# fema-ffrd/gpras

Hardware: AMD Instinct MI355X
Metric: gp_fits_per_sec (higher is better)
Workload: dtype f64; 1 GPU; BASELINE configs[1] as the many-independent-cells workload: exact GP N=4096 d=8 RBF, fit F1 = kernel build + blocked fp64-MFMA Cholesky + alpha + LML, per cell; cells = y columns of one training set with per-cell hyperparameters (the reference's per-mode models); n_train=4096, d=8, kernel=RBF, collective=none (one process), launcher=single process

## Files before the change

### gpras_amd/_lib.py

```python

from __future__ import annotations

import ctypes as C
from pathlib import Path

import numpy as np

import os

LIB_PATH = Path(os.environ["GPRX_LIBRARY"]) if os.environ.get("GPRX_LIBRARY") else Path(__file__).resolve().parent / "libgprx.so"

GPRX_OK, GPRX_EINVAL, GPRX_ENOTPD, GPRX_EHIP, GPRX_ENOMEM, GPRX_ESTATE, GPRX_ERCCL, GPRX_ENOCONV = range(8)
UNIQUE_ID_BYTES = 128
TRAIN_VARIANCE, TRAIN_LENGTHSCALE, TRAIN_NOISE, TRAIN_Z = 1, 2, 4, 8
GEMM_C_LOWER, GEMM_A_LOWER, GEMM_A_UPPER, GEMM_B_LOWER, GEMM_B_UPPER = 1, 2, 4, 8, 16
REDUCE_LOGDET_QUAD, REDUCE_COL, REDUCE_ROWSQ_FINAL, REDUCE_ROW = range(4)

DISTANCE_FORMS = {"difference": 0, "expanded": 1}
KERNEL_IDS = {"RBF": 0, "Matern12": 1, "Matern32": 2, "Matern52": 3, "Exponential": 4}


class GprxLibraryError(RuntimeError):
    """libgprx.so is missing or unusable."""

# ... 96 lines not shown
    "gprx_api": (C.c_int, [C.c_int, _vp, _i64, _vp, _i64, _i64, _vp]),
    "gprx_spline_eval": (C.c_int, [C.c_int, _vp, C.c_int, _vp, _vp, _i64, _vp]),
    "gprx_ps_create": (C.c_int, [C.c_int, _i64, _vp, _vp, _i64, _vp, _vp, C.c_int, _vp, _vp, C.c_int, _vp, C.POINTER(_vp)]),
    "gprx_ps_destroy": (C.c_int, [_vp]),
    "gprx_ps_last_error": (C.c_char_p, [_vp]),
    "gprx_ps_set_weights": (C.c_int, [_vp, _vp]),
    "gprx_ps_fit_centerline": (C.c_int, [_vp, _vp, _vp, _vp, _vp, _vp, _i64, _vp]),
    "gprx_ps_timings": (C.c_int, [_vp, _dp]),
    "gprx_ps_rating": (C.c_int, [_vp, _vp, _vp, _i64, _vp, _vp]),
    "gprx_ps_set_boundaries": (C.c_int, [_vp, _vp, _vp, _i64]),
    "gprx_ps_centerline": (C.c_int, [_vp, _vp]),
    "gprx_ps_gather": (C.c_int, [_vp, _vp, _i64, _vp]),
    "gprx_ps_surface": (C.c_int, [_vp, _vp, _vp]),
    "gprx_ps_surface_dev": (C.c_int, [_vp, _i64, _i64, _vp, _i64, _vp, _i64]),
    "gprx_ps_synchronize": (C.c_int, [_vp]),
    "gprx_pca_slab_rows": (C.c_int, [_vp, C.POINTER(_i64)]),
    "gprx_rs_create": (C.c_int, [C.c_int, _i64, _i64, C.c_int, _vp, _vp, _vp, C.POINTER(_vp)]),
    "gprx_rs_destroy": (C.c_int, [_vp]),
    "gprx_rs_last_error": (C.c_char_p, [_vp]),
    "gprx_rs_apply": (C.c_int, [_vp, _vp, _vp, _i64, _vp]),
    "gprx_rs_apply_dev": (C.c_int, [_vp, _i64, _vp, _i64, _vp, _vp, _i64]),
    "gprx_rs_synchronize": (C.c_int, [_vp]),
    "gprx_rs_timings": (C.c_int, [_vp, _dp]),
    "gprx_al_create": (C.c_int, [C.c_int, C.POINTER(_vp)]),
    "gprx_al_destroy": (C.c_int, [_vp]),
    "gprx_al_last_error": (C.c_char_p, [_vp]),
    "gprx_al_synchronize": (C.c_int, [_vp]),
    "gprx_al_cutoff_dev": (C.c_int, [_vp, C.c_int, _vp, _vp, _vp, _i64, C.c_double, C.POINTER(_i64), C.POINTER(_i64), C.POINTER(_i64), _vp]),
    "gprx_al_cutoff": (C.c_int, [_vp, _vp, _i64, _i64, C.c_double, C.POINTER(_i64), C.POINTER(_i64), C.POINTER(_i64), _vp]),
    "gprx_al_clip_dev": (C.c_int, [_vp, _vp, _i64, _i64, _i64, _i64, _vp, _i64]),
    "gprx_al_timings": (C.c_int, [_vp, _dp]),
    "gprx_dg_create": (C.c_int, [C.c_int, C.POINTER(_vp)]),
    "gprx_dg_destroy": (C.c_int, [_vp]),
    "gprx_dg_last_error": (C.c_char_p, [_vp]),
    "gprx_dg_synchronize": (C.c_int, [_vp]),
    "gprx_dg_sort_u64_dev": (C.c_int, [_vp, _vp, _i64, _vp]),
    "gprx_dg_sort_abs_residual_dev": (C.c_int, [_vp, _vp, _vp, _i64, _vp]),
    "gprx_dg_sort_info": (C.c_int, [_vp, _ip, _dp]),
    "gprx_dg_gather_dev": (C.c_int, [_vp, _vp, _i64, _vp, _i64, _vp]),
    "gprx_dg_scatter_summary_dev": (C.c_int, [_vp, _vp, _vp, _i64, _vp]),
    "gprx_dg_detect_dev": (C.c_int, [_vp, _vp, _vp, _i64, _i64, _vp, _vp, _i64, C.c_double, C.c_int, _vp, C.POINTER(_i64)]),
    "gprx_ev_create": (C.c_int, [C.c_int, _i64, _i64, _i64, _vp, _vp, _vp, _vp, _vp, C.POINTER(_vp)]),
    "gprx_ev_create_empty": (C.c_int, [C.c_int, C.POINTER(_vp)]),
    "gprx_ev_destroy": (C.c_int, [_vp]),
    "gprx_ev_last_error": (C.c_char_p, [_vp]),
    "gprx_ev_synchronize": (C.c_int, [_vp]),
    "gprx_ev_maxima": (C.c_int, [_vp, _vp, _vp, _vp]),
    "gprx_ev_return_periods": (C.c_int, [_vp, _i64, _vp, _vp, _vp]),
    "gprx_ev_rp_eval": (C.c_int, [_vp, C.c_int, _vp, _i64, _vp]),
    "gprx_ev_cov": (C.c_int, [_vp, C.c_int, _vp, _vp]),
    "gprx_ev_eigh": (C.c_int, [_vp, _vp, _vp, _ip]),
    "gprx_ev_scores": (C.c_int, [_vp, C.c_int, C.c_int, _vp]),
    "gprx_ev_standardise": (C.c_int, [_vp, _vp]),
    "gprx_ev_farthest": (C.c_int, [_vp, _vp, _i64, C.c_int, _vp, _i64, _i64, _vp, _vp]),
    "gprx_ev_timings": (C.c_int, [_vp, _dp]),
    "gprx_metrics": (C.c_int, [C.c_int, _vp, _vp, _vp, _i64, _i64, C.c_int, C.c_double, _vp, _vp, _vp, C.POINTER(C.c_uint64)]),
    "gprx_metrics_dev": (C.c_int, [C.c_int, _vp, _vp, _vp, _i64, _i64, C.c_int, C.c_double, _vp, _vp, _vp, C.POINTER(C.c_uint64)]),
    "gprx_kmeans_pp": (C.c_int, [C.c_int, _vp, _i64, C.c_int, _vp, C.c_int, C.c_int, _i64, _vp, _vp]),
    "gprx_kmeans_lloyd": (C.c_int, [C.c_int, _vp, _i64, C.c_int, _vp, C.c_int, C.c_double, C.c_int, _vp, _ip, _ip]),
    "gprx_gather_rows": (C.c_int, [C.c_int, _vp, _i64, _i64, _vp, _vp]),
    "gprx_kmat": (C.c_int, [C.c_int, C.c_int, _vp, _i64, _vp, _i64, C.c_int, _vp, C.c_double, C.c_double, _vp, _i64, _i64, _i64, C.c_int]),
    "gprx_gemm": (C.c_int, [C.c_int, C.c_int, C.c_int, _i64, _i64, _i64, C.c_double, _vp, _i64, _vp, _i64, C.c_double, _vp, _i64, C.c_int, C.c_int]),
    "gprx_potrf": (C.c_int, [C.c_int, _vp, _i64, _i64, _i64, _vp, _ip]),
    "gprx_gemm_batched": (C.c_int, [C.c_int, C.c_int, C.c_int, _i64, _i64, _i64, C.c_double, _vp, _i64, _vp, _i64, C.c_double, _vp, _i64, C.c_int, C.c_int,
                                    C.c_int, _i64, _i64, _i64, C.c_int, _i64, _i64, _i64, _vp, C.c_int, _vp, _i64]),
    "gprx_gemm_splitk": (C.c_int, [C.c_int, C.c_int, C.c_int, _i64, _i64, _i64, C.c_double, _vp, _i64, _vp, _i64, C.c_double, _vp, _i64, _vp, C.c_int,
                                   C.c_int, _i64, _i64, _i64, _i64, _vp, C.c_int]),
    "gprx_trsv_lower": (C.c_int, [C.c_int, _vp, _i64, _vp, _vp, _i64, C.c_int, C.c_int, _i64, _vp]),
    "gprx_potrf_batched": (C.c_int, [C.c_int, _vp, _i64, _i64, _i64, _vp, _vp, _vp, C.c_int, _i64, C.c_int, C.c_int, C.c_int, C.c_int, C.c_int, _ip]),
    "gprx_trsm_lower_left": (C.c_int, [C.c_int, _vp, _i64, _vp, _vp, _i64, _i64, _i64, C.c_int, _i64, _vp]),
    "gprx_trtri_lower": (C.c_int, [C.c_int, _vp, _i64, _vp, _vp, _i64, _vp, _i64, _i64, C.c_int, _i64, _i64, C.c_int]),
    "gprx_transpose_inplace": (C.c_int, [C.c_int, _vp, _i64, _i64, C.c_int, _i64]),
    "gprx_alpha_from_inverse": (C.c_int, [C.c_int, _vp, _i64, _vp, _vp, _vp, _i64, C.c_int, _i64, _i64, _i64]),
    "gprx_reduce_probe": (C.c_int, [C.c_int, C.c_int, _vp, _i64, _vp, _i64, _i64, C.c_double, C.c_double, C.c_int, _vp, C.c_int, _vp, C.c_int, _i64, _i64,
                                    _i64, _i64, _vp, _vp, C.c_int]),
    "gprx_set_tuning": (C.c_int, [C.c_char_p, C.c_int]),
    "gprx_set_handle_tuning": (C.c_int, [_vp, C.c_char_p, C.c_int]),
    "gprx_mfma_f64_peak": (C.c_int, [C.c_int, _dp]),
    "gprx_exp_probe": (C.c_int, [C.c_int, C.c_int, _vp, _i64, _vp]),
}

TUNING_KEYS = (
    "outer_block", "update_tile", "no_lookahead", "split_panel", "dag", "rhs_vector", "cell_kernel", "poison_workspace", "predict_path",
    "sgpr_fused", "sgpr_resident", "wait_handover_us", "sgpr_groups_from",
)

_lib = None


def load():
    global _lib
    if _lib is not None:
        return _lib
    if not LIB_PATH.exists():
        raise GprxLibraryError(
            f"{LIB_PATH} not found: build it with `python -c 'import __graft_entry__ as g; g.build()'` "
            "(hipcc --offload-arch=gfx950).  gpras_amd has no CPU fallback."
        )
    try:
        lib = C.CDLL(str(LIB_PATH))
    except OSError as exc:
        raise GprxLibraryError(f"cannot load {LIB_PATH}: {exc}") from exc
    for name, (res, args) in PROTOTYPES.items():
        try:
            fn = getattr(lib, name)
        except AttributeError as exc:
            raise GprxLibraryError(f"{LIB_PATH} does not export {name}") from exc
        fn.restype = res
        fn.argtypes = args
    _lib = lib
    return lib


def last_error(handle=None) -> str:
    msg = load().gprx_last_error(handle)
    return msg.decode() if msg else ""


def check(rc: int, handle=None) -> None:
    if rc == GPRX_OK:
        return
    msg = last_error(handle)
    if rc == GPRX_EINVAL:
        raise ValueError(msg)
    if rc == GPRX_ENOTPD:
        raise np.linalg.LinAlgError(msg)
    if rc == GPRX_ENOCONV:
        raise np.linalg.LinAlgError(msg)
    if rc == GPRX_ENOMEM:
        raise MemoryError(msg)
    raise RuntimeError(f"libgprx error {rc}: {msg}")


def as_f64(a) -> np.ndarray:
    return np.ascontiguousarray(a, dtype=np.float64)


def ptr(a: np.ndarray):
    return _vp(a.ctypes.data)


class DeviceBuffer:

    def __init__(self, nbytes: int, device: int = 0):
        self.device = device
        self.nbytes = int(nbytes)
        p = _vp()
        check(load().gprx_dev_malloc(device, self.nbytes, C.byref(p)))
        self.ptr = p

    @classmethod
    def from_array(cls, a, device: int = 0) -> "DeviceBuffer":
        a = as_f64(a)
        buf = cls(a.nbytes, device)
        check(load().gprx_memcpy_h2d(device, buf.ptr, ptr(a), a.nbytes))
        return buf

    def to_array(self, shape) -> np.ndarray:
        out = np.empty(shape, dtype=np.float64)
        assert out.nbytes <= self.nbytes
        check(load().gprx_memcpy_d2h(self.device, ptr(out), self.ptr, out.nbytes))
        return out

    def at(self, offset_elems: int):
        return _vp(self.ptr.value + 8 * int(offset_elems))

    def free(self):
# ... 10 lines not shown
```

### gpras_amd/csrc/gemm_f64.h

```cpp
#pragma once
#include <cstdlib>

#include "gprx_common.h"

namespace gprx {

struct GemmArgs {
  const double* A;
  const double* B;
  double* C;
  int64_t lda, ldb, ldc;
  int M, N, K;
  double alpha, beta;
  int flags;
  int tiles_n;
  int tiles_m;
  int nwg;
  int64_t strideA, strideB, strideC;
  int ksplit;
  int64_t slab;
  int inner = 0;
  int64_t cellA = 0, cellB = 0, cellC = 0;
  const double* a_sub = nullptr;
  const double* a_mul = nullptr;
  const double* a_elev = nullptr;
  const double* alpha_tab = nullptr;
  int alpha_stride = 0;
  double* rowsq = nullptr;
  int64_t rowsq_ld = 0;
  int cell_xcd = 0;
};

#ifndef GPRX_GEMM_PFC_DEFAULT
#define GPRX_GEMM_PFC_DEFAULT 1
#endif
#ifndef GPRX_GEMM_DMA_DEFAULT
#define GPRX_GEMM_DMA_DEFAULT 1
#endif
constexpr int GEMM_BK = 16;
constexpr int GEMM_LDK = GEMM_BK;
__device__ __forceinline__ int kc_swz(int row) { return (int)((0xa7a09f5366f7ull >> (3 * (row & 15))) & 7ull); }

template <int BMN>
struct McStride {
  static constexpr int value = BMN + 4;
};

template <int ROWS>
__device__ __forceinline__ void load_kc(d2 (&r)[ROWS / 32], const double* __restrict__ base, int64_t ld, int row0, int nrows_valid,
                                        int k0, int tid) {
#pragma unroll
  for (int i = 0; i < ROWS / 32; ++i) {
    const int q = tid + 256 * i;
    const int row = q >> 3, cc = q & 7;
    if (row0 + row < nrows_valid)
      r[i] = *reinterpret_cast<const d2*>(base + (int64_t)(row0 + row) * ld + k0 + cc * 2);
    else
      r[i] = d2{0.0, 0.0};
  }
}
template <int ROWS>
__device__ __forceinline__ void store_kc(double* s, const d2 (&r)[ROWS / 32], int tid) {
#pragma unroll
  for (int i = 0; i < ROWS / 32; ++i) {
    const int q = tid + 256 * i;
    const int row = q >> 3, cc = q & 7;
    *reinterpret_cast<d2*>(s + row * GEMM_LDK + ((cc ^ kc_swz(row)) * 2)) = r[i];
  }
}
template <int COLS>
__device__ __forceinline__ void load_mc(d2 (&r)[COLS / 32], const double* __restrict__ base, int64_t ld, int col0, int ncols_valid,
                                        int k0, int tid) {
#pragma unroll
  for (int i = 0; i < COLS / 32; ++i) {
    const int q = tid + 256 * i;
    const int krow = q / (COLS / 2), cc = q % (COLS / 2);
    const int col = col0 + cc * 2;
    if (col + 1 < ncols_valid) {
      r[i] = *reinterpret_cast<const d2*>(base + (int64_t)(k0 + krow) * ld + col);
    } else if (col < ncols_valid) {
      r[i] = d2{base[(int64_t)(k0 + krow) * ld + col], 0.0};
    } else {
      r[i] = d2{0.0, 0.0};
    }
  }
}
template <int COLS>
__device__ __forceinline__ void store_mc(double* s, const d2 (&r)[COLS / 32], int tid) {
#pragma unroll
  for (int i = 0; i < COLS / 32; ++i) {
    const int q = tid + 256 * i;
    const int krow = q / (COLS / 2), cc = q % (COLS / 2);
    *reinterpret_cast<d2*>(s + krow * McStride<COLS>::value + cc * 2) = r[i];
  }
}

__device__ __forceinline__ void glds16(const double* src, double* lds_wave_base) {
  __builtin_amdgcn_global_load_lds((const __attribute__((address_space(1))) void*)src, (__attribute__((address_space(3))) void*)lds_wave_base, 16, 0, 0);
}

template <int TA, int TB, int BM, int BN>
struct GemmSmem {
  static constexpr int A_ELEMS = TA ? GEMM_BK * McStride<BM>::value : BM * GEMM_LDK;
  static constexpr int B_ELEMS = TB ? BN * GEMM_LDK : GEMM_BK * McStride<BN>::value;
  static constexpr int doubles = 2 * (A_ELEMS + B_ELEMS);
};

template <int TA, int TB, int BM, int BN, int PF, int AXF, int DMA>
__device__ __forceinline__ void gemm_tile(GemmArgs p, const int bx_in, const int by_in, const int bz, double* __restrict__ smem) {
  int bx = bx_in, by = by_in;
  if (p.cell_xcd) {
    const int L = bx_in + p.nwg * by_in, slot = L >> 3;
    const int cq = slot / p.nwg;
    by = (L & 7) + 8 * cq;
    bx = slot - cq * p.nwg;
  }
  static_assert(!DMA || (AXF == 0 && (TA == 0 || BM == 64) && (TB == 1 || BN == 64)),
                "the LDS-DMA staging exists for k-contiguous operands and for m/n-contiguous operands of 64-wide tiles");
  constexpr int TM = BM / 32, TN = BN / 32;
  constexpr int A_ELEMS = GemmSmem<TA, TB, BM, BN>::A_ELEMS;
  constexpr int B_ELEMS = GemmSmem<TA, TB, BM, BN>::B_ELEMS;

  const int tid = threadIdx.x;
  const int lane = tid & 63;
  const int wave = tid >> 6;
  const int wm = wave >> 1, wn = wave & 1;
  const int g = lane >> 4, r = lane & 15;

  {
    int entry = by;
    if (p.inner > 0) {
      const int cell = entry / p.inner;
      entry -= cell * p.inner;
      p.A += (int64_t)cell * p.cellA;
      p.B += (int64_t)cell * p.cellB;
      p.C += (int64_t)cell * p.cellC;
      if (p.alpha_tab) p.alpha = p.alpha_tab[(int64_t)cell * p.alpha_stride];
    }
    p.A += (int64_t)entry * p.strideA;
    p.B += (int64_t)entry * p.strideB;
    p.C += (int64_t)entry * p.strideC;
  }
  int bid = bx;
  if (!p.cell_xcd && !(p.flags & (GEMM_A_LOWER | GEMM_A_UPPER | GEMM_B_LOWER | GEMM_B_UPPER))) {
    const int q = p.nwg >> 3, rr = p.nwg & 7, xcd = bid & 7, k = bid >> 3;
    bid = (xcd < rr ? xcd * (q + 1) : rr * (q + 1) + (xcd - rr) * q) + k;
  }
  int ti, tj;
  if (p.flags & GEMM_C_LOWER) {
#ifndef GPRX_BAND
#define GPRX_BAND 4
#endif
    constexpr int R = GPRX_BAND;
    const int tn = p.tiles_n;
    const int tri = tn * (tn + 1) / 2;
    if (bid < tri) {
      int b = (int)((sqrtf((float)(R + 1) * (R + 1) / 4.0f - (float)(R + 1) * R / 2.0f + (float)R * R / 4.0f + 2.0f * (float)bid) -
                     (float)(R + 1) / 2.0f + (float)R / 2.0f) / (float)R);
      if (b < 0) b = 0;
      auto S = [](int bb) { return R * R * bb * (bb - 1) / 2 + bb * R * (R + 1) / 2; };
      while (S(b + 1) <= bid) ++b;
      while (S(b) > bid) --b;
      int u = bid - S(b);
      const int r0 = R * b;
      const int h = (tn - r0 < R) ? tn - r0 : R;
      if (u < h * r0) {
        tj = u / h;
        ti = r0 + u % h;
      } else {
        u -= h * r0;
        int c = 0;
        while (u >= h - c) {
          u -= h - c;
          ++c;
        }
        tj = r0 + c;
        ti = r0 + c + u;
      }
    } else {
      const int rest = bid - tri;
      const int b2 = rest / (R * tn);
      const int u = rest - b2 * R * tn;
      const int left = p.tiles_m - tn - R * b2;
      const int h = left < R ? left : R;
      tj = u / h;
      ti = tn + R * b2 + u % h;
    }
  } else {
    const int tri = p.flags & (GEMM_A_LOWER | GEMM_A_UPPER | GEMM_B_LOWER | GEMM_B_UPPER);
    if (tri == GEMM_B_UPPER || tri == GEMM_B_LOWER) {
      const int cj = bid / p.tiles_m;
      ti = bid % p.tiles_m;
// ... 85 lines not shown
    if constexpr (TB == 1)
      store_kc<BN>(sb, rb, tid);
    else
      store_mc<BN>(sb, rb, tid);
  };

  const int swz = kc_swz(r);
  auto stage = [&](int k0, int buf) {
    const bool more = (k0 + GEMM_BK) < kend;
    if (more) gload(k0 + GEMM_BK);
    const double* sa = smem + buf * (A_ELEMS + B_ELEMS);
    const double* sb = sa + A_ELEMS;
    double fa[TM][4], fb[TN][4];
#pragma unroll
    for (int a = 0; a < TM; ++a) {
      const int row = wm * (BM / 2) + a * 16 + r;
      if constexpr (TA == 0) {
        const d2 lo = *reinterpret_cast<const d2*>(sa + row * GEMM_LDK + 2 * ((2 * g) ^ swz));
        const d2 hi = *reinterpret_cast<const d2*>(sa + row * GEMM_LDK + 2 * ((2 * g + 1) ^ swz));
        fa[a][0] = lo.x; fa[a][1] = lo.y; fa[a][2] = hi.x; fa[a][3] = hi.y;
      } else {
#pragma unroll
        for (int j = 0; j < 4; ++j) fa[a][j] = sa[(4 * g + j) * McStride<BM>::value + row];
      }
    }
#pragma unroll
    for (int b = 0; b < TN; ++b) {
      const int col = wn * (BN / 2) + b * 16 + r;
      if constexpr (TB == 1) {
        const d2 lo = *reinterpret_cast<const d2*>(sb + col * GEMM_LDK + 2 * ((2 * g) ^ swz));
        const d2 hi = *reinterpret_cast<const d2*>(sb + col * GEMM_LDK + 2 * ((2 * g + 1) ^ swz));
        fb[b][0] = lo.x; fb[b][1] = lo.y; fb[b][2] = hi.x; fb[b][3] = hi.y;
      } else {
#pragma unroll
        for (int j = 0; j < 4; ++j) fb[b][j] = sb[(4 * g + j) * McStride<BN>::value + col];
      }
    }
#pragma unroll
    for (int j = 0; j < 4; ++j)
#pragma unroll
      for (int a = 0; a < TM; ++a)
#pragma unroll
        for (int b = 0; b < TN; ++b) acc[a][b] = __builtin_amdgcn_mfma_f64_16x16x4f64(fa[a][j], fb[b][j], acc[a][b], 0, 0, 0);
    if (more) sstore(buf ^ 1);
    __syncthreads();
  };
  if constexpr (DMA != 0) {
    const int wave_u = __builtin_amdgcn_readfirstlane(wave);
    auto dma_fill = [&](int k0, int buf) {
      double* sa = smem + buf * (A_ELEMS + B_ELEMS);
      double* sb = sa + A_ELEMS;
      if constexpr (TA == 0) {
#pragma unroll
        for (int i = 0; i < BM / 32; ++i) {
          const int rbase = (i * 4 + wave_u) * 8;
          const int row = rbase + (lane >> 3);
          glds16(p.A + (int64_t)(m0 + row) * p.lda + k0 + 2 * ((lane & 7) ^ kc_swz(row)), sa + rbase * GEMM_LDK);
        }
      } else {
#pragma unroll
        for (int i = 0; i < 2; ++i) {
          const int rbase = (i * 4 + wave_u) * 2;
          const int row = rbase + (lane >> 5);
          glds16(p.A + (int64_t)(k0 + row) * p.lda + m0 + 2 * ((lane & 31) ^ (8 * ((row >> 2) & 1))), sa + rbase * BM);
        }
      }
      if constexpr (TB == 1) {
#pragma unroll
        for (int i = 0; i < BN / 32; ++i) {
          const int rbase = (i * 4 + wave_u) * 8;
          const int row = rbase + (lane >> 3);
          glds16(p.B + (int64_t)(n0 + row) * p.ldb + k0 + 2 * ((lane & 7) ^ kc_swz(row)), sb + rbase * GEMM_LDK);
        }
      } else {
#pragma unroll
        for (int i = 0; i < 2; ++i) {
          const int rbase = (i * 4 + wave_u) * 2;
          const int row = rbase + (lane >> 5);
          glds16(p.B + (int64_t)(k0 + row) * p.ldb + n0 + 2 * ((lane & 31) ^ (8 * ((row >> 2) & 1))), sb + rbase * BN);
        }
      }
    };
    const int swz_d = kc_swz(r);
    auto dma_stage = [&](int k0, int buf) {
      if (k0 + GEMM_BK < kend) dma_fill(k0 + GEMM_BK, buf ^ 1);
      const double* sa = smem + buf * (A_ELEMS + B_ELEMS);
      const double* sb = sa + A_ELEMS;
      double fa[TM][4], fb[TN][4];
#pragma unroll
      for (int a = 0; a < TM; ++a) {
        const int row = wm * (BM / 2) + a * 16 + r;
        if constexpr (TA == 0) {
          const d2 lo = *reinterpret_cast<const d2*>(sa + row * GEMM_LDK + 2 * ((2 * g) ^ swz_d));
          const d2 hi = *reinterpret_cast<const d2*>(sa + row * GEMM_LDK + 2 * ((2 * g + 1) ^ swz_d));
          fa[a][0] = lo.x; fa[a][1] = lo.y; fa[a][2] = hi.x; fa[a][3] = hi.y;
        } else {
          const int pos = 2 * ((row >> 1) ^ (8 * (g & 1))) + (row & 1);
#pragma unroll
          for (int j = 0; j < 4; ++j) fa[a][j] = sa[(4 * g + j) * BM + pos];
        }
      }
#pragma unroll
      for (int b = 0; b < TN; ++b) {
        const int col = wn * (BN / 2) + b * 16 + r;
        if constexpr (TB == 1) {
          const d2 lo = *reinterpret_cast<const d2*>(sb + col * GEMM_LDK + 2 * ((2 * g) ^ swz_d));
          const d2 hi = *reinterpret_cast<const d2*>(sb + col * GEMM_LDK + 2 * ((2 * g + 1) ^ swz_d));
          fb[b][0] = lo.x; fb[b][1] = lo.y; fb[b][2] = hi.x; fb[b][3] = hi.y;
        } else {
          const int pos = 2 * ((col >> 1) ^ (8 * (g & 1))) + (col & 1);
#pragma unroll
          for (int j = 0; j < 4; ++j) fb[b][j] = sb[(4 * g + j) * BN + pos];
        }
      }
#pragma unroll
      for (int j = 0; j < 4; ++j)
#pragma unroll
        for (int a = 0; a < TM; ++a)
#pragma unroll
          for (int b = 0; b < TN; ++b) acc[a][b] = __builtin_amdgcn_mfma_f64_16x16x4f64(fa[a][j], fb[b][j], acc[a][b], 0, 0, 0);
      __syncthreads();
    };
    if (kbeg < kend) {
      dma_fill(kbeg, 0);
      __syncthreads();
      for (int k0 = kbeg; k0 < kend; k0 += 2 * GEMM_BK) {
        dma_stage(k0, 0);
        if (k0 + GEMM_BK < kend) dma_stage(k0 + GEMM_BK, 1);
      }
    }
  } else if (kbeg < kend) {
    gload(kbeg);
    sstore(0);
    __syncthreads();
    for (int k0 = kbeg; k0 < kend; k0 += 2 * GEMM_BK) {
      stage(k0, 0);
      if (k0 + GEMM_BK < kend) stage(k0 + GEMM_BK, 1);
    }
  }

  const double alpha = p.alpha, beta = p.beta;
  if (p.rowsq) {
#pragma unroll
    for (int a = 0; a < TM; ++a)
#pragma unroll
      for (int q = 0; q < 4; ++q) {
        double ssq = 0.0;
#pragma unroll
        for (int b = 0; b < TN; ++b) {
          const int col = n0 + wn * (BN / 2) + b * 16 + r;
          const double v = col < p.N ? alpha * acc[a][b][q] : 0.0;
          ssq = __builtin_fma(v, v, ssq);
        }
        ssq += __shfl_xor(ssq, 1, 64);
        ssq += __shfl_xor(ssq, 2, 64);
        ssq += __shfl_xor(ssq, 4, 64);
        ssq += __shfl_xor(ssq, 8, 64);
        const int row = m0 + wm * (BM / 2) + a * 16 + g + 4 * q;
        if (r == 0 && row < p.M) p.rowsq[(int64_t)(2 * tj + wn) * p.rowsq_ld + row] = ssq;
      }
    return;
  }
#pragma unroll
  for (int a = 0; a < TM; ++a) {
    double cold[TN][4];
    if constexpr (kPrefetchC) {
#pragma unroll
      for (int b = 0; b < TN; ++b)
#pragma unroll
        for (int q = 0; q < 4; ++q) cold[b][q] = cpre[a][b][q];
    } else if (beta != 0.0) {
#pragma unroll
      for (int b = 0; b < TN; ++b) {
        const int col = n0 + wn * (BN / 2) + b * 16 + r;
#pragma unroll
        for (int q = 0; q < 4; ++q) {
          const int row = m0 + wm * (BM / 2) + a * 16 + g + 4 * q;
          cold[b][q] = (row < p.M && col < p.N) ? p.C[(int64_t)row * p.ldc + col] : 0.0;
        }
      }
    }
#pragma unroll
    for (int b = 0; b < TN; ++b) {
      const int col = n0 + wn * (BN / 2) + b * 16 + r;
#pragma unroll
      for (int q = 0; q < 4; ++q) {
        const int row = m0 + wm * (BM / 2) + a * 16 + g + 4 * q;
        if (row < p.M && col < p.N) {
          double v = alpha * acc[a][b][q];
          if (beta != 0.0) v = __builtin_fma(beta, cold[b][q], v);
          p.C[(int64_t)row * p.ldc + col] = v;
        }
      }
    }
  }
}

template <int TA, int TB, int BM, int BN, int PF = 0, int AXF = 0, int DMA = 0>
__global__ __launch_bounds__(256, (BM * BN >= 128 * 128) ? 2 : (((PF && !DMA) || AXF) ? 3 : 4)) void gemm_f64_kernel(GemmArgs p) {
  __shared__ __attribute__((aligned(16))) double smem[GemmSmem<TA, TB, BM, BN>::doubles];
  gemm_tile<TA, TB, BM, BN, PF, AXF, DMA>(p, (int)blockIdx.x, (int)blockIdx.y, (int)blockIdx.z, smem);
}

template <int TA, int TB, int BM, int BN>
inline hipError_t launch_gemm_t(hipStream_t st, GemmArgs p, int batch, int nsplit = 1) {
  p.tiles_m = (p.M + BM - 1) / BM;
  p.tiles_n = (p.N + BN - 1) / BN;
  if (p.tiles_m == 0 || p.tiles_n == 0) return hipSuccess;
  if (p.flags & GEMM_C_LOWER) {
    if (p.tiles_n > p.tiles_m) p.tiles_n = p.tiles_m;
    p.nwg = p.tiles_n * (p.tiles_n + 1) / 2 + (p.tiles_m - p.tiles_n) * p.tiles_n;
  } else {
    p.nwg = p.tiles_m * p.tiles_n;
  }
  {
    static const int cell_xcd = getenv("GPRX_CELL_XCD") ? atoi(getenv("GPRX_CELL_XCD")) : 1;
    p.cell_xcd = (cell_xcd && p.inner == 0 && nsplit == 1 && batch >= 8 && batch % 8 == 0 &&
                  !(p.flags & (GEMM_A_LOWER | GEMM_A_UPPER | GEMM_B_LOWER | GEMM_B_UPPER))) ? 1 : 0;
  }
  if constexpr (TA == 0 && TB == 1) {
    static const int dma = getenv("GPRX_GEMM_DMA") ? atoi(getenv("GPRX_GEMM_DMA")) : GPRX_GEMM_DMA_DEFAULT;
    static const int pfc = getenv("GPRX_GEMM_PFC") ? atoi(getenv("GPRX_GEMM_PFC")) : GPRX_GEMM_PFC_DEFAULT;
    if (dma && p.M % BM == 0 && p.N % BN == 0 && p.K % GEMM_BK == 0 && p.lda % 2 == 0 && p.ldb % 2 == 0) {
      const bool prefetch_c = BM * BN <= 64 * 64 && p.beta != 0.0 && nsplit == 1 && (pfc >= 2 || (pfc == 1 && p.K <= 128));
      if (prefetch_c)
        hipLaunchKernelGGL((gemm_f64_kernel<0, 1, (BM > 64 ? 64 : BM), (BN > 64 ? 64 : BN), 1, 0, 1>), dim3(p.nwg, batch, nsplit), dim3(256), 0, st, p);
      else
        hipLaunchKernelGGL((gemm_f64_kernel<0, 1, BM, BN, 0, 0, 1>), dim3(p.nwg, batch, nsplit), dim3(256), 0, st, p);
      return hipGetLastError();
    }
  }
  if constexpr (TA == 0 && TB == 0 && BM == 64 && BN == 64) {
    static const int dma_nn = getenv("GPRX_GEMM_DMA_NN") ? atoi(getenv("GPRX_GEMM_DMA_NN")) : 1;
    if (dma_nn && p.M % BM == 0 && p.N % BN == 0 && p.K % GEMM_BK == 0 && p.lda % 2 == 0 && p.ldb % 2 == 0 && nsplit == 1 &&
        (reinterpret_cast<uintptr_t>(p.A) & 15) == 0 && (reinterpret_cast<uintptr_t>(p.B) & 15) == 0 && p.strideA % 2 == 0 && p.strideB % 2 == 0 &&
        p.cellA % 2 == 0 && p.cellB % 2 == 0) {
      hipLaunchKernelGGL((gemm_f64_kernel<0, 0, 64, 64, 0, 0, 1>), dim3(p.nwg, batch, nsplit), dim3(256), 0, st, p);
      return hipGetLastError();
    }
  }
  if constexpr (TA == 1 && TB == 0 && BM == 64 && BN == 64) {
    static const int dma_tn = getenv("GPRX_GEMM_DMA_TN") ? atoi(getenv("GPRX_GEMM_DMA_TN")) : 1;
    if (dma_tn && p.M % BM == 0 && p.N % BN == 0 && p.K % GEMM_BK == 0 && p.lda % 2 == 0 && p.ldb % 2 == 0 && nsplit == 1 &&
        (reinterpret_cast<uintptr_t>(p.A) & 15) == 0 && (reinterpret_cast<uintptr_t>(p.B) & 15) == 0 && p.strideA % 2 == 0 && p.strideB % 2 == 0 &&
        p.cellA % 2 == 0 && p.cellB % 2 == 0) {
      hipLaunchKernelGGL((gemm_f64_kernel<1, 0, 64, 64, 0, 0, 1>), dim3(p.nwg, batch, nsplit), dim3(256), 0, st, p);
      return hipGetLastError();
    }
  }
  if (BM * BN <= 64 * 64 && p.beta != 0.0 && p.K <= 128 && nsplit == 1) {
    hipLaunchKernelGGL((gemm_f64_kernel<TA, TB, (BM > 64 ? 64 : BM), (BN > 64 ? 64 : BN), 1>), dim3(p.nwg, batch, nsplit), dim3(256), 0, st, p);
  } else {
    hipLaunchKernelGGL((gemm_f64_kernel<TA, TB, BM, BN, 0>), dim3(p.nwg, batch, nsplit), dim3(256), 0, st, p);
  }
  return hipGetLastError();
}

inline hipError_t launch_gemm(hipStream_t st, int ta, int tb, int M, int N, int K, double alpha, const double* A, int64_t lda,
                              const double* B, int64_t ldb, double beta, double* C, int64_t ldc, int flags, int tile = 0, int batch = 1,
                              int64_t strideA = 0, int64_t strideB = 0, int64_t strideC = 0, int cells = 1, int64_t cellA = 0,
                              int64_t cellB = 0, int64_t cellC = 0, const double* alpha_tab = nullptr, int alpha_stride = 0,
                              double* rowsq = nullptr, int64_t rowsq_ld = 0) {
  GemmArgs p{A, B, C, lda, ldb, ldc, M, N, K, alpha, beta, flags, 0, 0, 0, strideA, strideB, strideC, 0, 0};
  p.rowsq = rowsq;
  p.rowsq_ld = rowsq_ld;
  if (M <= 0 || N <= 0 || batch <= 0 || cells <= 0) return hipSuccess;
  if (cells > 1 || alpha_tab) {
    p.inner = batch;
    p.cellA = cellA;
    p.cellB = cellB;
    p.cellC = cellC;
    p.alpha_tab = alpha_tab;
    p.alpha_stride = alpha_stride;
    batch *= cells;
  }
  static const int force_tile = getenv("GPRX_FORCE_TILE") ? atoi(getenv("GPRX_FORCE_TILE")) : 0;
  if (force_tile) tile = force_tile;
  if (tile == 0) {
    const int64_t t128 = (int64_t)batch * ((M + 127) / 128) * ((N + 127) / 128) / ((flags & GEMM_C_LOWER) ? 2 : 1);
    tile = (t128 >= 1024) ? 128 : 64;
  }
#define GPRX_GEMM_CASE(TA_, TB_)                                                  \
  if (ta == TA_ && tb == TB_) {                                                   \
    if (tile == 128) return launch_gemm_t<TA_, TB_, 128, 128>(st, p, batch);      \
    return launch_gemm_t<TA_, TB_, 64, 64>(st, p, batch);                         \
  }
  GPRX_GEMM_CASE(0, 1)
  GPRX_GEMM_CASE(0, 0)
  GPRX_GEMM_CASE(1, 0)
#undef GPRX_GEMM_CASE
  return hipErrorInvalidValue;
}

static __global__ __launch_bounds__(256) void splitk_reduce_kernel(const double* __restrict__ ws, int nsplit, int M, int N, double beta,
                                                            double* __restrict__ C, int64_t ldc, int64_t ws_cell = 0, int64_t c_cell = 0) {
  ws += (int64_t)blockIdx.y * ws_cell;
  C += (int64_t)blockIdx.y * c_cell;
  const int64_t e = blockIdx.x * (int64_t)256 + threadIdx.x;
  if (e >= (int64_t)M * N) return;
  const int i = (int)(e / N), j = (int)(e % N);
  double s = 0.0;
  for (int z = 0; z < nsplit; ++z) s += ws[(int64_t)z * M * N + e];
  double* cp = C + (int64_t)i * ldc + j;
  *cp = (beta != 0.0) ? beta * (*cp) + s : s;
}

inline hipError_t launch_gemm_splitk(hipStream_t st, int ta, int tb, int M, int N, int K, double alpha, const double* A, int64_t lda,
// ... 51 lines not shown
```

### gpras_amd/csrc/gprx.hip

```cpp
#include "abi_common.h"

#include <algorithm>
#include <chrono>
#include <cmath>
#include <cstdio>
#include <cstdlib>
#include <cstring>
#include <limits>
#include <map>
#include <mutex>
#include <string>
#include <thread>
#include <vector>

#include "gemm_f64.h"
#include "gprx_common.h"
#include "grad.h"
#include "kmat.h"
#include "potrf.h"
#include "potrf_cell.h"
#include "potrf_dag.h"
#include "sgpr.h"
#include "sgpr_asm.h"
#include "sgpr_fused.h"
// ... 737 lines not shown
    HIPCHK(nullptr, hipGetLastError());
    HIPCHK(nullptr, hipStreamSynchronize(st));
    return GPRX_OK;
  });
}

extern "C" int gprx_dag_stamps(gprx_handle h, unsigned long long* out, int max_words, int* T, int* grid) {
  if (!h || !h->dag.stamps) return 0;
  const int n = (int)std::min<size_t>(h->dag.stamp_words, (size_t)max_words);
  hipStreamSynchronize(h->stream);
  copy_sync(out, h->dag.stamps, sizeof(unsigned long long) * n, hipMemcpyDeviceToHost);
  if (T) *T = h->dag.T;
  if (grid) *grid = h->dag.grid;
  return n;
}

#ifdef GPRX_CHAIN_STAMPS
extern "C" int gprx_chain_stamps(unsigned long long* out16) {
  hipMemcpyFromSymbol(out16, HIP_SYMBOL(gprx::g_chain_stamps), sizeof(unsigned long long) * 16);
  return 0;
}
#endif

#ifdef GPRX_PANEL_ACC
int gprx_panel_acc(unsigned long long* out8, int reset) {
  if (reset) {
    unsigned long long z[8] = {0};
    hipMemcpyToSymbol(HIP_SYMBOL(gprx::g_panel_acc), z, sizeof(z));
  }
  hipMemcpyFromSymbol(out8, HIP_SYMBOL(gprx::g_panel_acc), sizeof(unsigned long long) * 8);
  return 0;
}
#endif
#ifdef GPRX_CELL_ACC
int gprx_cell_acc(unsigned long long* out16, int reset) {
  if (reset) {
    unsigned long long z[16] = {0};
    hipMemcpyToSymbol(HIP_SYMBOL(gprx::g_cell_acc), z, sizeof(z));
  }
  hipMemcpyFromSymbol(out16, HIP_SYMBOL(gprx::g_cell_acc), sizeof(unsigned long long) * 16);
  return 0;
}
#endif
int gprx_sf_stamps(gprx_handle h, int enable, unsigned long long* out) {
  return guarded(h, [&]() -> int {
    if (!h) return fail(h, GPRX_EINVAL, "null handle");
    HIPCHK(h, hipSetDevice(h->device));
    HIPCHK(h, hipStreamSynchronize(h->stream));
    if (out && h->sf_stamps) HIPCHK(h, copy_sync(out, h->sf_stamps, sizeof(unsigned long long) * SF_STAMP_WORDS, hipMemcpyDeviceToHost));
    if (enable && !h->sf_stamps) {
      HIPCHK(h, hipMalloc((void**)&h->sf_stamps, sizeof(unsigned long long) * SF_STAMP_WORDS));
      HIPCHK(h, memset_sync(h->sf_stamps, 0, sizeof(unsigned long long) * SF_STAMP_WORDS));
      drop_graphs(h);
    } else if (!enable && h->sf_stamps) {
      HIPCHK(h, hipFree(h->sf_stamps));
      h->sf_stamps = nullptr;
      drop_graphs(h);
    }
    return GPRX_OK;
  });
}
#ifdef GPRX_PANEL_STAMPS
int gprx_panel_stamps(unsigned long long* out64) {
  hipMemcpyFromSymbol(out64, HIP_SYMBOL(gprx::g_panel_stamps), sizeof(unsigned long long) * 64);
  return 0;
}
#endif

namespace {
bool apply_tuning(PotrfTuning& t, int& predict_path, int& fused, int& resident, const std::string& k, int value) {
  if (k == "outer_block" && value >= 0 && value % 128 == 0) t.outer_block = value;
  else if (k == "update_tile" && (value == 0 || value == 64 || value == 128)) t.update_tile = value;
  else if (k == "no_lookahead") t.no_lookahead = value != 0;
  else if (k == "split_panel" && value >= -1 && value <= 1) t.split_panel = value;
  else if (k == "dag" && value >= -1 && value <= 1) t.dag = value;
  else if (k == "rhs_vector" && value >= -1 && value <= 1) t.rhs_vector = value;
  else if (k == "cell_kernel" && value >= -1 && value <= 1) t.cell_kernel = value;
  else if (k == "poison_workspace" && value >= 0 && value <= 1) t.poison_workspace = value;
  else if (k == "predict_path" && value >= 0 && value <= 2) predict_path = value;
  else if (k == "sgpr_fused" && value >= 0 && value <= 1) fused = value;
  else if (k == "sgpr_resident" && value >= 0 && value <= 1) resident = value;
  else if (k == "wait_handover_us" && value >= 0) wait_handover_us() = value;
  else if (k == "sgpr_groups_from" && value >= 0) sf_groups_from() = value;
  else return false;
  return true;
}
}

int gprx_set_tuning(const char* key, int value) {
  return guarded(nullptr, [&]() -> int {
    if (!key) return fail(nullptr, GPRX_EINVAL, "null key");
    if (!apply_tuning(potrf_tuning(), predict_path_tuning(), sgpr_fused_tuning(), sgpr_resident_tuning(), key, value)) return fail(nullptr, GPRX_EINVAL, "unknown tuning key or bad value");
    return GPRX_OK;
  });
}

int gprx_set_handle_tuning(gprx_handle h, const char* key, int value) {
  return guarded(h, [&]() -> int {
    if (!h || !key) return fail(h, GPRX_EINVAL, "null argument");
    const int fused_before = h->sgpr_fused;
    if (!apply_tuning(h->tune, h->predict_path, h->sgpr_fused, h->sgpr_resident, key, value)) return fail(h, GPRX_EINVAL, "unknown tuning key or bad value");
    if (hipSetDevice(h->device) == hipSuccess && hipStreamSynchronize(h->stream) == hipSuccess) drop_graphs(h);
    if (h->sgpr_fused != fused_before) {
      h->sarena_slots = 0;
      if (h->m != 0) h->factorized = false;
    }
    return GPRX_OK;
  });
}

int gprx_mfma_f64_peak(int device, double* tflops) {
  return guarded(nullptr, [&]() -> int {
    if (!tflops) return fail(nullptr, GPRX_EINVAL, "null argument");
    HIPCHK(nullptr, hipSetDevice(device));
    double* out = nullptr;
    HIPCHK(nullptr, hipMalloc((void**)&out, 64));
    hipEvent_t e0, e1;
    hipEventCreate(&e0);
    hipEventCreate(&e1);
    const int iters = 20000, blocks = 256 * 4;
    hipStream_t us = util_stream();
    hipLaunchKernelGGL(mfma_f64_peak_kernel, dim3(blocks), dim3(256), 0, us, out, 100);
    hipEventRecord(e0, us);
    hipLaunchKernelGGL(mfma_f64_peak_kernel, dim3(blocks), dim3(256), 0, us, out, iters);
    hipEventRecord(e1, us);
    hipError_t e = hipStreamSynchronize(us);
    float ms = 0.f;
    hipEventElapsedTime(&ms, e0, e1);
    hipEventDestroy(e0);
    hipEventDestroy(e1);
    hipFree(out);
    HIPCHK(nullptr, e);
    const double flops = (double)blocks * 4  * iters * 4  * 2048.0;
    *tflops = flops / (ms * 1e-3) / 1e12;
    return GPRX_OK;
  });
}

}
```

Before: 2297 fits/s.

## Add 3/4-stage LDS-DMA operand ring to the NT 64x64 fp64 GEMM

Adds a multi-stage LDS operand ring (3 or 4 buffers) to the NT LDS-DMA GEMM kernel on 64x64 tiles. Global-to-LDS loads run two or three k-steps ahead, and the waits use partial vmcnt counts instead of a full __syncthreads drain after each stage. By default, K>128 selects 3 stages. This is meant to hide memory latency in the trailing Cholesky updates, at the cost of more LDS per block and lower occupancy bounds.

```diff
diff --git a/gpras_amd/_lib.py b/gpras_amd/_lib.py
--- a/gpras_amd/_lib.py
+++ b/gpras_amd/_lib.py
@@ -202,7 +202,7 @@
 
 TUNING_KEYS = (
     "outer_block", "update_tile", "no_lookahead", "split_panel", "dag", "rhs_vector", "cell_kernel", "poison_workspace", "predict_path",
-    "sgpr_fused", "sgpr_resident", "wait_handover_us", "sgpr_groups_from",
+    "sgpr_fused", "sgpr_resident", "wait_handover_us", "sgpr_groups_from", "gemm_stages",
 )
 
 _lib = None
diff --git a/gpras_amd/csrc/gemm_f64.h b/gpras_amd/csrc/gemm_f64.h
--- a/gpras_amd/csrc/gemm_f64.h
+++ b/gpras_amd/csrc/gemm_f64.h
@@ -1,5 +1,6 @@
 #pragma once
 #include <cstdlib>
+#include <utility>
 
 #include "gprx_common.h"
 
@@ -99,15 +100,27 @@
   __builtin_amdgcn_global_load_lds((const __attribute__((address_space(1))) void*)src, (__attribute__((address_space(3))) void*)lds_wave_base, 16, 0, 0);
 }
 
-template <int TA, int TB, int BM, int BN>
+template <int TA, int TB, int BM, int BN, int NST = 2>
 struct GemmSmem {
   static constexpr int A_ELEMS = TA ? GEMM_BK * McStride<BM>::value : BM * GEMM_LDK;
   static constexpr int B_ELEMS = TB ? BN * GEMM_LDK : GEMM_BK * McStride<BN>::value;
-  static constexpr int doubles = 2 * (A_ELEMS + B_ELEMS);
+  static constexpr int doubles = NST * (A_ELEMS + B_ELEMS);
 };
 
-template <int TA, int TB, int BM, int BN, int PF, int AXF, int DMA>
+template <int... I, class F>
+__device__ __forceinline__ void static_for(std::integer_sequence<int, I...>, F&& f) {
+  (f(std::integral_constant<int, I>{}), ...);
+}
+
+template <int N>
+__device__ __forceinline__ void ring_sync() {
+  asm volatile("s_waitcnt vmcnt(%0)\n\ts_waitcnt lgkmcnt(0)\n\ts_barrier" ::"n"(N) : "memory");
+}
+
+template <int TA, int TB, int BM, int BN, int PF, int AXF, int DMA, int NST = 2>
 __device__ __forceinline__ void gemm_tile(GemmArgs p, const int bx_in, const int by_in, const int bz, double* __restrict__ smem) {
+  static_assert(NST == 2 || ((NST == 3 || NST == 4) && DMA != 0 && TA == 0 && TB == 1 && BM == 64 && BN == 64),
+                "the operand ring exists for the NT LDS-DMA kernel on 64 x 64 tiles");
   int bx = bx_in, by = by_in;
   if (p.cell_xcd) {
     const int L = bx_in + p.nwg * by_in, slot = L >> 3;
@@ -359,8 +372,7 @@
       }
     };
     const int swz_d = kc_swz(r);
-    auto dma_stage = [&](int k0, int buf) {
-      if (k0 + GEMM_BK < kend) dma_fill(k0 + GEMM_BK, buf ^ 1);
+    auto dma_compute = [&](int buf) {
       const double* sa = smem + buf * (A_ELEMS + B_ELEMS);
       const double* sb = sa + A_ELEMS;
       double fa[TM][4], fb[TN][4];
@@ -396,14 +408,47 @@
         for (int a = 0; a < TM; ++a)
 #pragma unroll
           for (int b = 0; b < TN; ++b) acc[a][b] = __builtin_amdgcn_mfma_f64_16x16x4f64(fa[a][j], fb[b][j], acc[a][b], 0, 0, 0);
-      __syncthreads();
     };
-    if (kbeg < kend) {
-      dma_fill(kbeg, 0);
-      __syncthreads();
-      for (int k0 = kbeg; k0 < kend; k0 += 2 * GEMM_BK) {
-        dma_stage(k0, 0);
-        if (k0 + GEMM_BK < kend) dma_stage(k0 + GEMM_BK, 1);
+    if constexpr (NST == 2) {
+      auto dma_stage = [&](int k0, int buf) {
+        if (k0 + GEMM_BK < kend) dma_fill(k0 + GEMM_BK, buf ^ 1);
+        dma_compute(buf);
+        __syncthreads();
+      };
+      if (kbeg < kend) {
+        dma_fill(kbeg, 0);
+        __syncthreads();
+        for (int k0 = kbeg; k0 < kend; k0 += 2 * GEMM_BK) {
+          dma_stage(k0, 0);
+          if (k0 + GEMM_BK < kend) dma_stage(k0 + GEMM_BK, 1);
+        }
+      }
+    } else {
+      constexpr int PER = BM / 32 + BN / 32;
+      auto ring_wait = [&](int rem) {
+        if (rem >= NST - 1) ring_sync<PER * (NST - 2)>();
+        else if (NST == 4 && rem == 2) ring_sync<PER>();
+        else if (rem >= 1) ring_sync<0>();
+      };
+      auto ring_stage = [&](auto buf_c, auto steady_c, int k0) {
+        constexpr int buf = decltype(buf_c)::value;
+        constexpr bool steady = decltype(steady_c)::value;
+        if (steady || k0 + (NST - 1) * GEMM_BK < kend) dma_fill(k0 + (NST - 1) * GEMM_BK, (buf + NST - 1) % NST);
+        dma_compute(buf);
+        if constexpr (steady) ring_sync<PER * (NST - 2)>();
+        else ring_wait((kend - k0) / GEMM_BK - 1);
+      };
+      if (kbeg < kend) {
+        static_for(std::make_integer_sequence<int, NST - 1>{}, [&](auto i) {
+          if (kbeg + i.value * GEMM_BK < kend) dma_fill(kbeg + i.value * GEMM_BK, i.value);
+        });
+        ring_wait((kend - kbeg) / GEMM_BK);
+        int k0 = kbeg;
+        for (; k0 + (2 * NST - 2) * GEMM_BK < kend; k0 += NST * GEMM_BK)
+          static_for(std::make_integer_sequence<int, NST>{}, [&](auto i) { ring_stage(i, std::true_type{}, k0 + i.value * GEMM_BK); });
+        static_for(std::make_integer_sequence<int, 2 * NST - 2>{}, [&](auto t) {
+          if (k0 + t.value * GEMM_BK < kend) ring_stage(std::integral_constant<int, decltype(t)::value % NST>{}, std::false_type{}, k0 + t.value * GEMM_BK);
+        });
       }
     }
   } else if (kbeg < kend) {
@@ -473,10 +518,23 @@
   }
 }
 
-template <int TA, int TB, int BM, int BN, int PF = 0, int AXF = 0, int DMA = 0>
-__global__ __launch_bounds__(256, (BM * BN >= 128 * 128) ? 2 : (((PF && !DMA) || AXF) ? 3 : 4)) void gemm_f64_kernel(GemmArgs p) {
-  __shared__ __attribute__((aligned(16))) double smem[GemmSmem<TA, TB, BM, BN>::doubles];
-  gemm_tile<TA, TB, BM, BN, PF, AXF, DMA>(p, (int)blockIdx.x, (int)blockIdx.y, (int)blockIdx.z, smem);
+template <int TA, int TB, int BM, int BN, int PF = 0, int AXF = 0, int DMA = 0, int NST = 2>
+__global__ __launch_bounds__(256, NST == 4 ? 2 : NST == 3 ? 3 : (BM * BN >= 128 * 128) ? 2 : (((PF && !DMA) || AXF) ? 3 : 4)) void gemm_f64_kernel(GemmArgs p) {
+  __shared__ __attribute__((aligned(16))) double smem[GemmSmem<TA, TB, BM, BN, NST>::doubles];
+  gemm_tile<TA, TB, BM, BN, PF, AXF, DMA, NST>(p, (int)blockIdx.x, (int)blockIdx.y, (int)blockIdx.z, smem);
+}
+
+inline int& gemm_stages_tuning() {
+  static int v = [] {
+    const int e = getenv("GPRX_GEMM_STAGES") ? atoi(getenv("GPRX_GEMM_STAGES")) : 0;
+    return (e >= 2 && e <= 4) ? e : 0;
+  }();
+  return v;
+}
+inline int gemm_stages_for(int K) {
+  const int forced = gemm_stages_tuning();
+  if (forced) return forced;
+  return K <= 128 ? 2 : K <= 512 ? 3 : 3;
 }
 
 template <int TA, int TB, int BM, int BN>
@@ -500,6 +558,17 @@
     static const int pfc = getenv("GPRX_GEMM_PFC") ? atoi(getenv("GPRX_GEMM_PFC")) : GPRX_GEMM_PFC_DEFAULT;
     if (dma && p.M % BM == 0 && p.N % BN == 0 && p.K % GEMM_BK == 0 && p.lda % 2 == 0 && p.ldb % 2 == 0) {
       const bool prefetch_c = BM * BN <= 64 * 64 && p.beta != 0.0 && nsplit == 1 && (pfc >= 2 || (pfc == 1 && p.K <= 128));
+      if constexpr (BM == 64 && BN == 64) {
+        const int nst = gemm_stages_for(p.K);
+        if (nst > 2) {
+          const dim3 grid(p.nwg, batch, nsplit);
+          if (prefetch_c && nst == 3) hipLaunchKernelGGL((gemm_f64_kernel<0, 1, 64, 64, 1, 0, 1, 3>), grid, dim3(256), 0, st, p);
+          else if (prefetch_c) hipLaunchKernelGGL((gemm_f64_kernel<0, 1, 64, 64, 1, 0, 1, 4>), grid, dim3(256), 0, st, p);
+          else if (nst == 3) hipLaunchKernelGGL((gemm_f64_kernel<0, 1, 64, 64, 0, 0, 1, 3>), grid, dim3(256), 0, st, p);
+          else hipLaunchKernelGGL((gemm_f64_kernel<0, 1, 64, 64, 0, 0, 1, 4>), grid, dim3(256), 0, st, p);
+          return hipGetLastError();
+        }
+      }
       if (prefetch_c)
         hipLaunchKernelGGL((gemm_f64_kernel<0, 1, (BM > 64 ? 64 : BM), (BN > 64 ? 64 : BN), 1, 0, 1>), dim3(p.nwg, batch, nsplit), dim3(256), 0, st, p);
       else
diff --git a/gpras_amd/csrc/gprx.hip b/gpras_amd/csrc/gprx.hip
--- a/gpras_amd/csrc/gprx.hip
+++ b/gpras_amd/csrc/gprx.hip
@@ -843,6 +843,7 @@
   else if (k == "sgpr_resident" && value >= 0 && value <= 1) resident = value;
   else if (k == "wait_handover_us" && value >= 0) wait_handover_us() = value;
   else if (k == "sgpr_groups_from" && value >= 0) sf_groups_from() = value;
+  else if (k == "gemm_stages" && (value == 0 || (value >= 2 && value <= 4))) gemm_stages_tuning() = value;
   else return false;
   return true;
 }
```

After: 2313 fits/s, median of 6. No clear change (+0.7%).
